# nkkrnkl/category-agnostic-pose-estimation

Hardware: AMD Instinct MI355X
Metric: episodes/sec (1-shot, 256x256, 17kpt) training step (higher is better)
Workload: dtype f32 storage/accumulate, GEMMs as bf16x3 split (3 bf16 MFMAs per product); 1 GPU; configs[1]: 1-shot training step (fwd+loss+bwd+clip+AdamW at learning rate 0, dropout on), 256x256, 17 kpt, ResNet-50 + deformable transformer, 16 episodes x 2 queries per GPU; episodes_per_gpu=16, queries_per_episode=2, image_size=256, global_batch_episodes=16, parallelism=dp1, weights=random init (no checkpoint offline)

## Files before the change

category-agnostic-pose-estimation_amd/csrc/msda.hip:

```cpp
#include <stdlib.h>
#include "common.h"

namespace {

struct Levels {
  int H[4], W[4], start[4];
};

constexpr int HEADS = 8, HD = 32, CH = HEADS * HD;

__device__ __forceinline__ int sel4(const int (&a)[4], int l) { return l == 0 ? a[0] : (l == 1 ? a[1] : (l == 2 ? a[2] : a[3])); }

__global__ void __launch_bounds__(256) msda_fwd_kernel(const float* __restrict__ value, const float* __restrict__ offw,
                                                        const float* __restrict__ ref, float* __restrict__ out,
                                                        Levels lv, int N, int S, int Lq, int L, int P, int blocks_per_image) {
  const int lane = threadIdx.x & 63, wv = threadIdx.x >> 6;
  int n, chunk;
  {
    const int b = blockIdx.x;
    const int xcd = b & 7, loc = b >> 3;
    const int imgs_per_x = (N + 7) >> 3;
    const int ii = loc / blocks_per_image;
    chunk = loc - ii * blocks_per_image;
    n = ii * 8 + xcd;
// ... 363 lines not shown
      const float top = v00.C + fx * dt, bot = v10.C + fx * db;                    \
      p_aw += go.C * (top + fy * (bot - top));                                     \
      p_x += go.C * (dt + fy * (db - dt));                                         \
      p_y += go.C * (bot - top);                                                   \
    }
    CAPE_TAP_CH(x) CAPE_TAP_CH(y) CAPE_TAP_CH(z) CAPE_TAP_CH(w)
#undef CAPE_TAP_CH
    const float r_aw = sum8(p_aw), r_x = sum8(p_x), r_y = sum8(p_y);
    if (i == (j & 7)) { daw[j >> 3] = r_aw; dpx[j >> 3] = r_x; dpy[j >> 3] = r_y; }
  }
  const float dot = sum8(aw[0] * daw[0] + aw[1] * daw[1]);
  float* dow = d_offw + qrow * rowlen;
#pragma unroll
  for (int s = 0; s < 2; ++s) {
    const int j = i + 8 * s;
    const bool live = j < LP;
    const float gx = aw[s] * dpx[s], gy = aw[s] * dpy[s];
    if (live) {
      *reinterpret_cast<float2*>(dow + (h * LP + j) * 2) = make_float2(gx, gy);
      dow[HEADS * LP * 2 + h * LP + j] = aw[s] * (daw[s] - dot);
    }
    if (d_ref) {
      float rx = live ? gx * (float)sel4(lv.W, lev[s]) : 0.f;
      float ry = live ? gy * (float)sel4(lv.H, lev[s]) : 0.f;
      if (P == 4) {
        rx += dpp_f<0xB1>(rx); rx += dpp_f<0x4E>(rx);
        ry += dpp_f<0xB1>(ry); ry += dpp_f<0x4E>(ry);
        rx += __shfl_xor(rx, 8); rx += __shfl_xor(rx, 16); rx += __shfl_xor(rx, 32);
        ry += __shfl_xor(ry, 8); ry += __shfl_xor(ry, 16); ry += __shfl_xor(ry, 32);
        if (live && h == 0 && (i & 3) == 0) *reinterpret_cast<float2*>(&d_ref[(qrow * L + lev[s]) * 2]) = make_float2(rx, ry);
      } else if (live) {
        atomicAdd(&d_ref[(qrow * L + lev[s]) * 2 + 0], rx);
        atomicAdd(&d_ref[(qrow * L + lev[s]) * 2 + 1], ry);
      }
    }
  }
}

struct ValRec { uint2 ids; float4 w; };

template <int VC>
__global__ void __launch_bounds__(1024) msda_bwd_value_kernel(const float* __restrict__ d_out, const float* __restrict__ offw,
                                                              const float* __restrict__ ref, float* __restrict__ d_value,
                                                              Levels lv, int N, int S, int Lq, int L, int P) {
  constexpr int VS = VC, GROUPS = HD / VC, BPI = HEADS * GROUPS;
  constexpr int SLOTS = 64 / VC;
  extern __shared__ __attribute__((aligned(16))) double slab[];
  __shared__ uint2 rec_ids[16][64];
  __shared__ float4 rec_w[16][64];
  int n, sub;
  {
    const int b = blockIdx.x, xcd = b & 7, loc = b >> 3;
    n = (loc / BPI) * 8 + xcd;
    sub = loc % BPI;
    if (n >= N) return;
  }
  const int h = sub / GROUPS, grp = sub % GROUPS;
  for (int k = threadIdx.x; k < (S + 1) * VS; k += 1024) slab[k] = 0.0;
  __syncthreads();

  const int lane = threadIdx.x & 63, wv = threadIdx.x >> 6;
  const int g = lane >> 4, j = lane & 15;
  const int c = lane & (VC - 1), slot = lane / VC;
  static_assert(SLOTS * VC == 64 && 16 % VC == 0, "a slot's records must stay inside one query");
  const int LP = L * P;
  const int rowlen = HEADS * LP * 3;
// ... 182 lines not shown
    const int l = (int)(unsigned)wd;
    const int hh = (int)(unsigned)(wd >> 32) - (l >> 31);
    lo = finite ? (float)l * inv_scale : nanv;
    hi = finite ? (float)hh * inv_scale : nanv;
  };
  constexpr int Q = VP / 2;
  for (int k = threadIdx.x; k < S * Q; k += 1024) {
    const int p_ = k / Q, c2 = (k % Q) * 2;
    float4 o;
    dec(fslab[p_ * VP + c2], o.x, o.y);
    dec(fslab[p_ * VP + c2 + 1], o.z, o.w);
    *reinterpret_cast<float4*>(dvb + (long long)p_ * CH + c2 * 2) = o;
  }
}

int fill_levels(Levels& lv, const int* shapes, const int* level_start, int L, int S) {
  CAPE_REQUIRE(L >= 1 && L <= 4, "cape_msda: L=%d must be in 1..4", L);
  long long tot = 0;
  for (int l = 0; l < 4; ++l) {
    lv.H[l] = l < L ? shapes[2 * l] : 1;
    lv.W[l] = l < L ? shapes[2 * l + 1] : 1;
    lv.start[l] = l < L ? level_start[l] : 0;
    if (l < L) {
      CAPE_REQUIRE(lv.H[l] > 0 && lv.W[l] > 0 && lv.start[l] == tot, "cape_msda: level %d shape/start inconsistent", l);
      tot += (long long)lv.H[l] * lv.W[l];
    }
  }
  CAPE_REQUIRE(tot == S, "cape_msda: sum(H*W)=%lld != S=%d", tot, S);
  return 0;
}

}

extern "C" int cape_msda_fwd(const float* value, const float* offw, const float* ref, const int* shapes,
                             const int* level_start, float* out, int N, int S, int Lq, int L, int P,
                             cape_stream_t stream) {
  CAPE_REQUIRE(value && offw && ref && shapes && level_start && out, "cape_msda_fwd: null pointer");
  CAPE_REQUIRE(P >= 1 && L * P <= 16, "cape_msda_fwd: L*P=%d must be <= 16", L * P);
  if (N <= 0 || Lq <= 0) return 0;
  Levels lv;
  if (fill_levels(lv, shapes, level_start, L, S)) return 1;
  const int bpi = (Lq + 3) / 4;
  const int imgs_per_x = (N + 7) / 8;
  const long long blocks = (long long)imgs_per_x * bpi * 8;
  CAPE_REQUIRE(blocks < (1ll << 31), "cape_msda_fwd: grid too large");
  static const bool shuffle_form = getenv("CAPE_MSDA_FWD_SHUFFLE") != nullptr;
  if (S < 65535 && !shuffle_form)
    hipLaunchKernelGGL(msda_fwd_rec_kernel, dim3((unsigned)blocks), dim3(256), 0, as_stream(stream), value, offw, ref, out, lv,
                       N, S, Lq, L, P, bpi);
  else
    hipLaunchKernelGGL(msda_fwd_kernel, dim3((unsigned)blocks), dim3(256), 0, as_stream(stream), value, offw, ref, out, lv,
                       N, S, Lq, L, P, bpi);
  CAPE_LAUNCH_CHECK("cape_msda_fwd");
  return 0;
}

static int msda_bwd_check(const float* d_out, const float* value, const float* offw, const float* ref, const int* shapes,
                          const int* level_start, float* d_value, float* d_offw, int L, int P) {
  CAPE_REQUIRE(d_out && value && offw && ref && shapes && level_start && d_value && d_offw, "cape_msda_bwd: null pointer");
  CAPE_REQUIRE(P >= 1 && L * P <= 16, "cape_msda_bwd: L*P=%d must be <= 16", L * P);
  return 0;
}

extern "C" int cape_msda_bwd_atomic(const float* d_out, const float* value, const float* offw, const float* ref,
                                    const int* shapes, const int* level_start, float* d_value, float* d_offw, float* d_ref,
                                    int N, int S, int Lq, int L, int P, cape_stream_t stream) {
  if (msda_bwd_check(d_out, value, offw, ref, shapes, level_start, d_value, d_offw, L, P)) return 1;
  if (N <= 0 || Lq <= 0) return 0;
  Levels lv;
  if (fill_levels(lv, shapes, level_start, L, S)) return 1;
  hipError_t e = hipMemsetAsync(d_value, 0, sizeof(float) * (size_t)N * S * CH, as_stream(stream));
  if (e == hipSuccess && d_ref) e = hipMemsetAsync(d_ref, 0, sizeof(float) * (size_t)N * Lq * L * 2, as_stream(stream));
  if (e != hipSuccess) return cape_set_error("cape_msda_bwd_atomic: memset: %s", hipGetErrorString(e));
  const long long waves = (long long)N * Lq * 4;
  const long long blocks = (waves + 3) / 4;
  CAPE_REQUIRE(blocks < (1ll << 31), "cape_msda_bwd_atomic: grid too large");
  hipLaunchKernelGGL(msda_bwd_kernel, dim3((unsigned)blocks), dim3(256), 0, as_stream(stream), d_out, value, offw, ref,
                     d_value, d_offw, d_ref, lv, N, S, Lq, L, P, waves);
  CAPE_LAUNCH_CHECK("cape_msda_bwd_atomic");
  return 0;
}

extern "C" int cape_msda_bwd(const float* d_out, const float* value, const float* offw, const float* ref,
                             const int* shapes, const int* level_start, float* d_value, float* d_offw, float* d_ref,
                             int N, int S, int Lq, int L, int P, cape_stream_t stream) {
  return cape_msda_bwd_ex(d_out, value, offw, ref, shapes, level_start, d_value, d_offw, d_ref, N, S, Lq, L, P, 0, stream);
}

extern "C" int cape_msda_bwd_ex(const float* d_out, const float* value, const float* offw, const float* ref,
                                const int* shapes, const int* level_start, float* d_value, float* d_offw, float* d_ref,
                                int N, int S, int Lq, int L, int P, int value_accum, cape_stream_t stream) {
  CAPE_REQUIRE(value_accum == 0 || value_accum == 1, "cape_msda_bwd_ex: value_accum must be 0 (fp64 slab) or 1 (fixed-point pairs)");
  if (msda_bwd_check(d_out, value, offw, ref, shapes, level_start, d_value, d_offw, L, P)) return 1;
  if (N <= 0 || Lq <= 0) return 0;
  const size_t kMaxSlab = 160 * 1024 - 16 * 64 * (sizeof(uint4) + sizeof(float4)) - 512;
  int vc = 8;
  while (vc >= 2 && (size_t)(S + 1) * vc * sizeof(double) > kMaxSlab) vc >>= 1;
  const size_t slab_bytes = (size_t)(S + 1) * vc * sizeof(double);
  static const bool force_atomic = getenv("CAPE_MSDA_BWD_ATOMIC") != nullptr;
  const long long imgs8 = ((long long)N + 7) / 8;
  const int bpi = (Lq + 3) / 4;
  const long long vblocks = imgs8 * 8 * HEADS * (HD / (vc < 2 ? 2 : vc));
  if (force_atomic || vc < 2 || S >= 65535 || vblocks >= (1ll << 31) || imgs8 * 8 * bpi >= (1ll << 31))
    return cape_msda_bwd_atomic(d_out, value, offw, ref, shapes, level_start, d_value, d_offw, d_ref, N, S, Lq, L, P, stream);
  Levels lv;
  if (fill_levels(lv, shapes, level_start, L, S)) return 1;
  static bool attr_done = false;
  if (!attr_done) {
    hipError_t e = hipFuncSetAttribute(reinterpret_cast<const void*>(msda_bwd_value_kernel<8>),
                                       hipFuncAttributeMaxDynamicSharedMemorySize, (int)kMaxSlab);
    if (e == hipSuccess) e = hipFuncSetAttribute(reinterpret_cast<const void*>(msda_bwd_value_kernel<4>),
                                                 hipFuncAttributeMaxDynamicSharedMemorySize, (int)kMaxSlab);
    if (e == hipSuccess) e = hipFuncSetAttribute(reinterpret_cast<const void*>(msda_bwd_value_kernel<2>),
                                                 hipFuncAttributeMaxDynamicSharedMemorySize, (int)kMaxSlab);
    if (e == hipSuccess) e = hipFuncSetAttribute(reinterpret_cast<const void*>(msda_bwd_value_fx_kernel<8>),
                                                 hipFuncAttributeMaxDynamicSharedMemorySize, (int)kMaxSlab);
    if (e == hipSuccess) e = hipFuncSetAttribute(reinterpret_cast<const void*>(msda_bwd_value_fx_kernel<4>),
                                                 hipFuncAttributeMaxDynamicSharedMemorySize, (int)kMaxSlab);
    if (e == hipSuccess) e = hipFuncSetAttribute(reinterpret_cast<const void*>(msda_bwd_value_fx_kernel<2>),
                                                 hipFuncAttributeMaxDynamicSharedMemorySize, (int)kMaxSlab);
    if (e != hipSuccess) return cape_set_error("cape_msda_bwd: hipFuncSetAttribute: %s", hipGetErrorString(e));
    attr_done = true;
  }
  if (d_ref && P != 4) {
    hipError_t e = hipMemsetAsync(d_ref, 0, sizeof(float) * (size_t)N * Lq * L * 2, as_stream(stream));
    if (e != hipSuccess) return cape_set_error("cape_msda_bwd: memset: %s", hipGetErrorString(e));
  }
#define VALUE_LAUNCH(W)                                                                                                     \
  hipLaunchKernelGGL((msda_bwd_value_kernel<W>), dim3((unsigned)vblocks), dim3(1024), slab_bytes, as_stream(stream), d_out, offw, \
                     ref, d_value, lv, N, S, Lq, L, P)
#define VALUE_LAUNCH_FX(W)                                                                                                  \
  hipLaunchKernelGGL((msda_bwd_value_fx_kernel<W>), dim3((unsigned)fxblocks), dim3(1024), fx_bytes, as_stream(stream),           \
                     d_out, offw, ref, d_value, lv, N, S, Lq, L, P)
  if (value_accum == 1) {
    int vp = vc;
    while (vp > 2 && imgs8 * 8 * HEADS * (HD / (2 * vp)) < 256) vp >>= 1;
    const long long fxblocks = imgs8 * 8 * HEADS * (HD / (2 * vp));
    const size_t fx_bytes = (size_t)(S + 1) * vp * sizeof(unsigned long long);
    if (vp == 8) VALUE_LAUNCH_FX(8); else if (vp == 4) VALUE_LAUNCH_FX(4); else VALUE_LAUNCH_FX(2);
  } else {
    if (vc == 8) VALUE_LAUNCH(8); else if (vc == 4) VALUE_LAUNCH(4); else VALUE_LAUNCH(2);
  }
#undef VALUE_LAUNCH_FX
#undef VALUE_LAUNCH
  hipLaunchKernelGGL(msda_bwd_offw_kernel, dim3((unsigned)(imgs8 * 8 * bpi)), dim3(256), 0, as_stream(stream), d_out, value, offw,
                     ref, d_offw, d_ref, lv, N, S, Lq, L, P, bpi);
  CAPE_LAUNCH_CHECK("cape_msda_bwd");
  return 0;
}
```

category-agnostic-pose-estimation_amd/hip/lib.py:

```python
import ctypes
import os

import torch

from ctypes import POINTER, c_char_p, c_float, c_int, c_int32, c_int64, c_longlong, c_size_t, c_uint32, c_uint64, c_uint8, c_void_p

_HERE = os.path.dirname(os.path.abspath(__file__))
LIB_PATH = os.environ.get("CAPE_HIP_LIB", os.path.join(_HERE, "..", "csrc", "libcape_hip.so"))
LIB_PATH = os.path.abspath(LIB_PATH)

if not os.path.exists(LIB_PATH):
    raise ImportError(
        f"libcape_hip.so not found at {LIB_PATH}; build it with `python -c 'import __graft_entry__ as g; g.build()'` "
        "(or `make -C category-agnostic-pose-estimation_amd/csrc`).  There is no CPU fallback.")
try:
    _lib = ctypes.CDLL(LIB_PATH)
except OSError as e:
    raise ImportError(f"cannot load {LIB_PATH}: {e}") from e

_lib.cape_last_error.restype = c_char_p
_lib.cape_abi_version.restype = c_int


class GemmDesc(ctypes.Structure):
# ... 67 lines not shown
        "w_off", "b_off", "value", "w_mo", "b_mo", "ln1_g", "ln1_b",
        "w1", "b1", "w2", "b2", "ln3_g", "ln3_b", "m1w", "m1b", "m2w", "m2b", "m3w", "m3b")]


class DecodeStepDesc(ctypes.Structure):
    _fields_ = [
        ("N", c_int), ("n_layers", c_int), ("step", c_int), ("T", c_int), ("P", c_int), ("S", c_int), ("L", c_int),
        ("n_points", c_int), ("ncls", c_int), ("ffn_dim", c_int),
        ("shapes", c_int * 8), ("level_start", c_int * 4),
        ("emb", c_void_p), ("qpos0", c_void_p), ("refin0", c_void_p), ("ref0", c_void_p), ("vr", c_void_p), ("dim_t", c_void_p),
        ("class_w", c_void_p), ("class_b", c_void_p),
        ("pos_w", c_void_p), ("pos_b", c_void_p), ("pos_gamma", c_void_p), ("pos_beta", c_void_p),
        ("out_logits", c_void_p), ("ld_logits", c_longlong),
        ("out_coords", c_void_p), ("ld_coords", c_longlong),
        ("out_hs", c_void_p), ("ld_hs", c_longlong),
        ("layers", DecodeLayerDesc * DECODE_MAX_LAYERS),
    ]


P, I, LL, F, U32 = c_void_p, c_int, c_longlong, c_float, c_uint32
_SIGS = {
    "cape_rng_advance": [P, P],
    "cape_stream_fork": [P, P],
    "cape_stream_join": [P, P],
    "cape_gemm_f32": [POINTER(GemmDesc), P],
    "cape_gemm_group_f32": [POINTER(GemmDesc), I, I, P],
    "cape_pack_weights": [P, I, I, P],
    "cape_colsum_f32": [P, LL, I, LL, I, I, P, I, P],
    "cape_add_layernorm_fwd": [P, P, P, P, P, P, P, P, P, I, I, F, P, U32, P],
    "cape_add_layernorm_bwd": [P, P, P, P, P, P, P, P, P, P, P, I, I, F, P, U32, P],
    "cape_groupnorm_fwd": [P, P, P, P, LL, P, P, I, I, I, I, P, c_size_t, P],
    "cape_groupnorm_bwd": [P, LL, P, P, P, P, P, P, P, I, I, I, I, P, c_size_t, P],
    "cape_msda_fwd": [P, P, P, P, P, P, I, I, I, I, I, P],
    "cape_msda_bwd": [P, P, P, P, P, P, P, P, P, I, I, I, I, I, P],
    "cape_msda_bwd_ex": [P, P, P, P, P, P, P, P, P, I, I, I, I, I, I, P],
    "cape_msda_bwd_atomic": [P, P, P, P, P, P, P, P, P, I, I, I, I, I, P],
    "cape_attn_fwd": [P, P, P, P, P, LL, LL, LL, LL, LL, LL, LL, LL, I, I, I, I, F, I, I, P, F, P, U32, P],
    "cape_attn_bwd": [P, P, P, P, P, P, P, P, P, LL, LL, LL, LL, LL, LL, LL, LL, I, I, I, I, F, I, I, P, F, P, U32, P],
    "cape_flash_attn_fwd": [P, P, P, P, P, LL, LL, LL, LL, LL, LL, LL, LL, I, I, I, I, F, I, I, P, F, P, U32, P],
    "cape_flash_attn_bwd": [P, P, P, P, P, P, P, P, P, P, LL, LL, LL, LL, LL, LL, LL, LL, I, I, I, I, F, I, I, P, F, P, U32, P],
    "cape_attn_softmax_fwd": [P, P, P, I, I, I, I, F, I, I, P, F, P, U32, P],
    "cape_attn_softmax_bwd": [P, P, I, I, I, I, F, F, P, U32, P],
    "cape_add_f32": [P, P, P, LL, P],
    "cape_level_embed_add": [P, P, P, P, I, I, I, I, P],
    "cape_add_n_f32": [POINTER(c_void_p), I, P, LL, P],
    "cape_add_n_rows_f32": [POINTER(c_void_p), POINTER(c_longlong), I, P, LL, LL, I, P],
    "cape_augment_batch": [P, I, I, I, P, P, P],
    "cape_gelu_f32": [P, P, LL, P],
    "cape_support_masks": [P, P, P, I, I, I, P],
    "cape_interleave2x2_f32": [POINTER(c_void_p), P, P, I, I, I, I, P],
    "cape_gelu_bwd_f32": [P, P, P, LL, P],
    "cape_scale_residual_bwd_f32": [P, P, P, P, P, LL, I, P],
    "cape_scale_residual_f32": [P, P, P, P, LL, I, P],
    "cape_nchw_to_nhwc": [P, P, I, I, I, I, I, P],
    "cape_bn_fold": [P, P, P, P, F, P, P, I, P],
    "cape_maxpool3x3s2_nhwc": [P, P, I, I, I, I, P],
    "cape_bn_relu_bwd": [P, P, P, P, P, LL, I, I, P],
    "cape_affine_act_f32": [P, P, P, P, LL, I, I, P],
    "cape_relu_drop_bwd": [P, P, P, LL, F, P],
    "cape_pos_sine_level": [P, P, P, P, LL, I, I, I, I, P],
    "cape_token_embed_fwd": [P, P, P, P, P, P, P, P, P, P, LL, I, I, P],
    "cape_token_embed_bwd": [P, P, P, P, P, P, P, P, P, P, LL, I, I, I, P],
    "cape_query_sine_fwd": [P, P, P, LL, P],
    "cape_query_sine_bwd": [P, P, P, P, I, LL, P],
    "cape_refine_fwd": [P, P, P, LL, P],
    "cape_refine_bwd": [P, P, P, P, P, I, LL, P],
    "cape_sigmoid_fwd": [P, P, LL, P],
    "cape_sigmoid_bwd": [P, P, P, I, LL, P],
# ... 55 lines not shown
```

category-agnostic-pose-estimation_amd/hip/ops.py:

```python
import ctypes
import math
import os
import weakref

import torch

from . import lib

_F32 = torch.float32


_raw_stream = getattr(torch._C, "_cuda_getCurrentRawStream", None)
_raw_device = getattr(torch._C, "_cuda_getDevice", None)


_side = [None]


def raw_current_stream():
    if _raw_stream is not None and _raw_device is not None:
        return _raw_stream(_raw_device())
    return torch.cuda.current_stream().cuda_stream


# ... 400 lines not shown
    assert x.numel() == N * HW * C
    mean = torch.empty(N * G, dtype=_F32, device=x.device)
    rstd = torch.empty(N * G, dtype=_F32, device=x.device)
    ws, nbytes = _gn_workspace(N, C, G, x.device)
    lib.call("cape_groupnorm_fwd", _p(x), _p(gamma), _p(beta), _p(out), out_image_stride, _p(mean), _p(rstd), N, HW, C, G,
             _p(ws), nbytes, _stream())
    return mean, rstd


def groupnorm_bwd(d_out, d_out_image_stride, x, gamma, mean, rstd, dgamma, dbeta, N, HW, C, G=32):
    _chk(d_out, "gn_bwd.d_out", contiguous=False)
    d_x = torch.empty_like(x)
    ws, nbytes = _gn_workspace(N, C, G, x.device)
    lib.call("cape_groupnorm_bwd", _p(d_out), d_out_image_stride, _p(x), _p(gamma), _p(mean), _p(rstd), _p(d_x),
             _p(dgamma), _p(dbeta), N, HW, C, G, _p(ws), nbytes, _stream())
    return d_x


class LevelGeometry:

    def __init__(self, shapes):
        self.shapes = [(int(h), int(w)) for h, w in shapes]
        self.L = len(self.shapes)
        starts, s = [], 0
        for h, w in self.shapes:
            starts.append(s)
            s += h * w
        self.S = s
        self.starts = starts
        self._shapes_c = (ctypes.c_int * (2 * self.L))(*[v for hw in self.shapes for v in hw])
        self._starts_c = (ctypes.c_int * self.L)(*starts)


def msda_fwd(value, offw, ref, geo, N, Lq, P=4):
    for t, n in ((value, "value"), (offw, "offw"), (ref, "ref")):
        _chk(t, "msda." + n)
    assert value.numel() == N * geo.S * 256 and offw.numel() == N * Lq * 8 * geo.L * P * 3
    assert ref.numel() == N * Lq * geo.L * 2
    out = torch.empty(N, Lq, 256, dtype=_F32, device=value.device)
    lib.call("cape_msda_fwd", _p(value), _p(offw), _p(ref), geo._shapes_c, geo._starts_c, _p(out), N, geo.S, Lq, geo.L, P,
             _stream())
    return out


MSDA_VALUE_ACCUM = os.environ.get("CAPE_MSDA_VALUE_ACCUM", "auto")


def msda_bwd(d_out, value, offw, ref, geo, N, Lq, P=4, need_ref_grad=True, form="split"):
    _chk(d_out, "msda_bwd.d_out")
    d_value = torch.empty_like(value)
    d_offw = torch.empty_like(offw)
    d_ref = torch.empty_like(ref) if need_ref_grad else None
    if form == "split":
        form = MSDA_VALUE_ACCUM if MSDA_VALUE_ACCUM != "auto" else ("f64" if GEMM_PRECISION == 0 else "fx")
    if form == "atomic":
        lib.call("cape_msda_bwd_atomic", _p(d_out), _p(value), _p(offw), _p(ref), geo._shapes_c, geo._starts_c, _p(d_value),
                 _p(d_offw), _p(d_ref), N, geo.S, Lq, geo.L, P, _stream())
    else:
        lib.call("cape_msda_bwd_ex", _p(d_out), _p(value), _p(offw), _p(ref), geo._shapes_c, geo._starts_c, _p(d_value),
                 _p(d_offw), _p(d_ref), N, geo.S, Lq, geo.L, P, {"f64": 0, "fx": 1}[form], _stream())
    return d_value, d_offw, d_ref


def _ld(t):
    assert t.stride(-1) == 1
    return t.stride(-2)


def _attn_views(tag, Q, K, V, N, H, Lq, Lk, flash):
    for t, n, L_ in ((Q, "Q", Lq), (K, "K", Lk), (V, "V", Lk)):
        _chk(t, tag + "." + n, contiguous=False)
        assert t.dim() == 3 and t.shape[0] == N and t.shape[1] >= L_ and t.shape[2] == H * 32
        if flash:
            assert t.stride(2) == 1 and t.stride(1) % 4 == 0 and t.stride(0) % 4 == 0 and t.data_ptr() % 16 == 0
        assert _avail(t) >= (N - 1) * t.stride(0) + (L_ - 1) * t.stride(1) + H * 32


def _rng_ptr(rng, dropout_p):
    return rng.ptr if (rng is not None and dropout_p > 0) else None


def _attn_tail(Q, K, V, N, H, Lq, Lk, scale, mask_mode, causal_offset, kpm, dropout_p, rng, rng_stream):
    return (_ld(Q), _ld(K), _ld(V), H * 32, Q.stride(0), K.stride(0), V.stride(0), Lq * H * 32, N, H, Lq, Lk, float(scale), mask_mode,
            causal_offset, _p(kpm), float(dropout_p), _rng_ptr(rng, dropout_p), rng_stream, _stream())


def _attn_fwd(flash, Q, K, V, N, H, Lq, Lk, scale, mask_mode, causal_offset, kpm, dropout_p, rng, rng_stream):
    tag = "flash_attn" if flash else "attn"
    _attn_views(tag, Q, K, V, N, H, Lq, Lk, flash)
    if kpm is not None:
        _chk(kpm, tag + ".kpm", dtype=torch.uint8)
        assert kpm.numel() == N * Lk
    O = torch.empty(N, Lq, H * 32, dtype=_F32, device=Q.device)
# ... 765 lines not shown
```

include/cape_hip.h:

```cpp
#ifndef CAPE_HIP_H
#define CAPE_HIP_H

#include <stddef.h>
#include <stdint.h>

#ifdef __cplusplus
extern "C" {
#endif

typedef void* cape_stream_t;

const char* cape_last_error(void);
int cape_abi_version(void);

int cape_rng_advance(uint64_t* rng_state, cape_stream_t stream);

int cape_stream_fork(cape_stream_t main_stream, cape_stream_t side_stream);
int cape_stream_join(cape_stream_t main_stream, cape_stream_t side_stream);

typedef struct {
  int M, N, K;
  int a_mode, b_mode;
  const float* A; long long lda;
  const float* B; long long ldb;
// ... 85 lines not shown
  const float* vr;
  const float* dim_t;
  const float *class_w, *class_b;
  const float *pos_w, *pos_b, *pos_gamma, *pos_beta;
  float* out_logits; long long ld_logits;
  float* out_coords; long long ld_coords;
  float* out_hs; long long ld_hs;
  cape_decode_layer_desc layers[CAPE_DECODE_MAX_LAYERS];
} cape_decode_step_desc;
int cape_decode_step(const cape_decode_step_desc* d, cape_stream_t stream);

int cape_add_layernorm_fwd(const float* x, const float* y, const float* gamma, const float* beta,
                           float* out, float* mean, float* rstd, const float* pos, float* out_pos,
                           int rows, int C, float dropout_p, const uint64_t* rng_state, uint32_t rng_stream,
                           cape_stream_t stream);
int cape_add_layernorm_bwd(const float* d_out, const float* d_out_pos, const float* x, const float* y,
                           const float* gamma, const float* mean, const float* rstd,
                           float* d_x, float* d_y, float* dgamma, float* dbeta,
                           int rows, int C, float dropout_p, const uint64_t* rng_state, uint32_t rng_stream,
                           cape_stream_t stream);

size_t cape_groupnorm_workspace_bytes(int N, int C, int G);
int cape_groupnorm_fwd(const float* x, const float* gamma, const float* beta, float* out,
                       long long out_image_stride, float* mean, float* rstd,
                       int N, int HW, int C, int G, void* workspace, size_t workspace_bytes, cape_stream_t stream);
int cape_groupnorm_bwd(const float* d_out, long long d_out_image_stride, const float* x,
                       const float* gamma, const float* mean, const float* rstd,
                       float* d_x, float* dgamma, float* dbeta, int N, int HW, int C, int G,
                       void* workspace, size_t workspace_bytes, cape_stream_t stream);

int cape_msda_fwd(const float* value, const float* offw, const float* ref, const int* shapes,
                  const int* level_start, float* out, int N, int S, int Lq, int L, int P,
                  cape_stream_t stream);
int cape_msda_bwd(const float* d_out, const float* value, const float* offw, const float* ref,
                  const int* shapes, const int* level_start, float* d_value, float* d_offw, float* d_ref,
                  int N, int S, int Lq, int L, int P, cape_stream_t stream);
int cape_msda_bwd_ex(const float* d_out, const float* value, const float* offw, const float* ref,
                     const int* shapes, const int* level_start, float* d_value, float* d_offw, float* d_ref,
                     int N, int S, int Lq, int L, int P, int value_accum, cape_stream_t stream);
int cape_msda_bwd_atomic(const float* d_out, const float* value, const float* offw, const float* ref,
                         const int* shapes, const int* level_start, float* d_value, float* d_offw, float* d_ref,
                         int N, int S, int Lq, int L, int P, cape_stream_t stream);

int cape_attn_fwd(const float* Q, const float* K, const float* V, float* O, float* lse,
                  long long ldq, long long ldk, long long ldv, long long ldo,
                  long long bsq, long long bsk, long long bsv, long long bso,
                  int N, int H, int Lq, int Lk, float scale, int mask_mode, int causal_offset,
                  const uint8_t* kpm, float dropout_p, const uint64_t* rng_state, uint32_t rng_stream,
                  cape_stream_t stream);
int cape_attn_bwd(const float* dO, const float* Q, const float* K, const float* V, const float* O,
                  const float* lse, float* dQ, float* dK, float* dV,
                  long long ldq, long long ldk, long long ldv, long long ldo,
                  long long bsq, long long bsk, long long bsv, long long bso,
                  int N, int H, int Lq, int Lk, float scale, int mask_mode, int causal_offset,
                  const uint8_t* kpm, float dropout_p, const uint64_t* rng_state, uint32_t rng_stream,
                  cape_stream_t stream);
int cape_attn_softmax_fwd(const float* S, float* P, float* Pd, int N, int H, int Lq, int Lk, float scale, int mask_mode,
                          int causal_offset, const uint8_t* kpm, float dropout_p, const uint64_t* rng_state,
                          uint32_t rng_stream, cape_stream_t stream);
int cape_attn_softmax_bwd(const float* P, float* dS, int N, int H, int Lq, int Lk, float scale, float dropout_p,
                          const uint64_t* rng_state, uint32_t rng_stream, cape_stream_t stream);

int cape_flash_attn_fwd(const float* Q, const float* K, const float* V, float* O, float* lse, long long ldq, long long ldk,
                        long long ldv, long long ldo, long long bsq, long long bsk, long long bsv, long long bso, int N, int H,
                        int Lq, int Lk, float scale, int mask_mode, int causal_offset, const uint8_t* kpm, float dropout_p,
                        const uint64_t* rng_state, uint32_t rng_stream, cape_stream_t stream);
int cape_flash_attn_bwd(const float* dO, const float* Q, const float* K, const float* V, const float* O, const float* lse,
                        float* dQ, float* dK, float* dV, float* d_ws, long long ldq, long long ldk, long long ldv, long long ldo,
                        long long bsq, long long bsk, long long bsv, long long bso, int N, int H, int Lq, int Lk, float scale,
                        int mask_mode, int causal_offset, const uint8_t* kpm, float dropout_p, const uint64_t* rng_state,
                        uint32_t rng_stream, cape_stream_t stream);

// ... 129 lines not shown
```

Baseline: 654.4 episodes/s.

## Add LDS-slab gather kernels for MSDA forward and offset-weight backward

Adds forward and offset/attention-weight backward kernels that stage the coarse levels of the value tensor for one (image, head) into shared memory. Taps on those levels are then read from LDS, while the finer levels are still gathered from global memory. A planner picks the split level under an LDS budget and sizes query chunks to fill the grid. The forward routes automatically when Lq is large enough and no reference gradient is needed. The backward slab path stays opt-in through an environment variable, and the change costs LDS occupancy plus extra launch-planning code.

```diff
diff --git a/category-agnostic-pose-estimation_amd/csrc/msda.hip b/category-agnostic-pose-estimation_amd/csrc/msda.hip
--- a/category-agnostic-pose-estimation_amd/csrc/msda.hip
+++ b/category-agnostic-pose-estimation_amd/csrc/msda.hip
@@ -419,6 +419,269 @@
       } else if (live) {
         atomicAdd(&d_ref[(qrow * L + lev[s]) * 2 + 0], rx);
         atomicAdd(&d_ref[(qrow * L + lev[s]) * 2 + 1], ry);
+      }
+    }
+  }
+}
+
+constexpr int SLAB_THREADS = 512, SLAB_WAVES = SLAB_THREADS / 64, SLAB_QPT = 8;
+constexpr int SLAB_STRIDE = 36;
+constexpr int GB = 4, GBB = 1;
+constexpr size_t SLAB_BUDGET = 52 * 1024;
+
+struct SlabGeo { int l0, row0, rows, ng, chunks, qchunk; };
+
+__device__ __forceinline__ bool slab_block(int N, const SlabGeo& sg, int& n, int& h, int& chunk) {
+  const int b = blockIdx.x, xcd = b & 7, loc = b >> 3;
+  const int per_img = HEADS * sg.chunks;
+  const int ii = loc / per_img, rem = loc - ii * per_img;
+  h = rem / sg.chunks;
+  chunk = rem - h * sg.chunks;
+  n = ii * 8 + xcd;
+  return n < N;
+}
+
+__device__ __forceinline__ void slab_fill(float* slab, const float* __restrict__ value, int n, int h, int S, const SlabGeo& sg) {
+  const float* src = value + ((long long)n * S + sg.row0) * CH + h * HD;
+  for (int k = threadIdx.x; k < sg.rows * 8; k += SLAB_THREADS) {
+    const int r = k >> 3, c = k & 7;
+    *reinterpret_cast<float4*>(slab + r * SLAB_STRIDE + c * 4) = *reinterpret_cast<const float4*>(src + (long long)r * CH + c * 4);
+  }
+  if (threadIdx.x < 8) *reinterpret_cast<float4*>(slab + sg.rows * SLAB_STRIDE + threadIdx.x * 4) = make_float4(0.f, 0.f, 0.f, 0.f);
+  __syncthreads();
+}
+
+__device__ __forceinline__ unsigned slab_id(unsigned id, bool in_slab, int S, const SlabGeo& sg) {
+  return in_slab ? (id >= (unsigned)S ? (unsigned)sg.rows : id - (unsigned)sg.row0) : id;
+}
+
+__global__ void __launch_bounds__(SLAB_THREADS) __attribute__((amdgpu_waves_per_eu(4, 4))) msda_fwd_slab_kernel(const float* __restrict__ value, const float* __restrict__ offw,
+                                                                     const float* __restrict__ ref, float* __restrict__ out,
+                                                                     Levels lv, SlabGeo sg, int N, int S, int Lq, int L, int P) {
+  extern __shared__ __attribute__((aligned(16))) float vslab[];
+  __shared__ uint2 rec_ids[SLAB_WAVES][SLAB_QPT * 16];
+  __shared__ float4 rec_w[SLAB_WAVES][SLAB_QPT * 16];
+  int n, h, chunk;
+  if (!slab_block(N, sg, n, h, chunk)) return;
+  slab_fill(vslab, value, n, h, S, sg);
+  const int lane = threadIdx.x & 63, wv = threadIdx.x >> 6;
+  const int qs = lane >> 3, i = lane & 7;
+  const int LP = L * P;
+  const int qend = min(Lq, (chunk + 1) * sg.qchunk);
+  int W[2], H[2], st[2], lev[2];
+#pragma unroll
+  for (int s = 0; s < 2; ++s) {
+    const int j = i + 8 * s;
+    lev[s] = j < LP ? j / P : 0;
+    W[s] = j < LP ? sel4(lv.W, lev[s]) : 1; H[s] = j < LP ? sel4(lv.H, lev[s]) : 1; st[s] = j < LP ? sel4(lv.start, lev[s]) : 0;
+  }
+  const float* vb = value + (long long)n * S * CH + h * HD + i * 4;
+  const float* sb = vslab + i * 4;
+  const uint2* rid = &rec_ids[wv][qs * 16];
+  const float4* rw = &rec_w[wv][qs * 16];
+  for (int qb = chunk * sg.qchunk + wv * SLAB_QPT; qb < qend; qb += SLAB_WAVES * SLAB_QPT) {
+    const int q = qb + qs;
+    const long long qrow = (long long)n * Lq + min(q, Lq - 1);
+    const float* ow = offw + qrow * (HEADS * LP * 3);
+    float px[2], py[2], lg[2];
+#pragma unroll
+    for (int s = 0; s < 2; ++s) {
+      const int j = i + 8 * s;
+      px[s] = 0.f; py[s] = 0.f; lg[s] = -INFINITY;
+      if (j < LP) {
+        const float2 rr = *reinterpret_cast<const float2*>(ref + (qrow * L + lev[s]) * 2);
+        const float2 oo = *reinterpret_cast<const float2*>(ow + (h * LP + j) * 2);
+        const float Wf = (float)W[s], Hf = (float)H[s];
+        px[s] = (rr.x + oo.x / Wf) * Wf - 0.5f;
+        py[s] = (rr.y + oo.y / Hf) * Hf - 0.5f;
+        lg[s] = ow[HEADS * LP * 2 + h * LP + j];
+      }
+    }
+    const float mx = max8(fmaxf(lg[0], lg[1]));
+    const float e0 = __expf(lg[0] - mx), e1 = __expf(lg[1] - mx);
+    const float inv = 1.f / sum8(e0 + e1);
+    const float aw[2] = {e0 * inv, e1 * inv};
+#pragma unroll
+    for (int s = 0; s < 2; ++s) {
+      const int j = i + 8 * s;
+      const Tap t = make_tap(px[s], py[s], W[s], H[s], st[s], j < LP, S);
+      const bool in_slab = j >= sg.ng;
+      const unsigned cl = (unsigned)(S - 1);
+      float4 w = make_float4(aw[s] * (1.f - t.fx) * (1.f - t.fy), aw[s] * t.fx * (1.f - t.fy), aw[s] * (1.f - t.fx) * t.fy,
+                             aw[s] * t.fx * t.fy);
+      if (t.i00 >= (unsigned)S) w.x = 0.f;
+      if (t.i01 >= (unsigned)S) w.y = 0.f;
+      if (t.i10 >= (unsigned)S) w.z = 0.f;
+      if (t.i11 >= (unsigned)S) w.w = 0.f;
+      const unsigned a = in_slab ? slab_id(t.i00, true, S, sg) : min(t.i00, cl), b = in_slab ? slab_id(t.i01, true, S, sg) : min(t.i01, cl);
+      const unsigned c = in_slab ? slab_id(t.i10, true, S, sg) : min(t.i10, cl), d = in_slab ? slab_id(t.i11, true, S, sg) : min(t.i11, cl);
+      rec_ids[wv][qs * 16 + j] = make_uint2(a | (b << 16), c | (d << 16));
+      rec_w[wv][qs * 16 + j] = w;
+    }
+    float4 acc = make_float4(0.f, 0.f, 0.f, 0.f);
+    auto consume = [&](const float4& w, const float4& c0, const float4& c1, const float4& c2, const float4& c3) {
+      acc.x += w.x * c0.x + w.y * c1.x + w.z * c2.x + w.w * c3.x;
+      acc.y += w.x * c0.y + w.y * c1.y + w.z * c2.y + w.w * c3.y;
+      acc.z += w.x * c0.z + w.y * c1.z + w.z * c2.z + w.w * c3.z;
+      acc.w += w.x * c0.w + w.y * c1.w + w.z * c2.w + w.w * c3.w;
+    };
+    auto sload = [&](int j, float4& w, float4 (&c)[4]) {
+      const uint2 ids = rid[j];
+      c[0] = *reinterpret_cast<const float4*>(sb + (ids.x & 0xFFFFu) * (unsigned)SLAB_STRIDE);
+      c[1] = *reinterpret_cast<const float4*>(sb + (ids.x >> 16) * (unsigned)SLAB_STRIDE);
+      c[2] = *reinterpret_cast<const float4*>(sb + (ids.y & 0xFFFFu) * (unsigned)SLAB_STRIDE);
+      c[3] = *reinterpret_cast<const float4*>(sb + (ids.y >> 16) * (unsigned)SLAB_STRIDE);
+      w = rw[j];
+    };
+    float4 cw, cc[4];
+    for (int j0 = 0; j0 < sg.ng; j0 += GB) {
+      float4 v[GB][4];
+#pragma unroll
+      for (int k = 0; k < GB; ++k) {
+        const uint2 ids = rid[min(j0 + k, sg.ng - 1)];
+        v[k][0] = *reinterpret_cast<const float4*>(vb + (ids.x & 0xFFFFu) * (unsigned)CH);
+        v[k][1] = *reinterpret_cast<const float4*>(vb + (ids.x >> 16) * (unsigned)CH);
+        v[k][2] = *reinterpret_cast<const float4*>(vb + (ids.y & 0xFFFFu) * (unsigned)CH);
+        v[k][3] = *reinterpret_cast<const float4*>(vb + (ids.y >> 16) * (unsigned)CH);
+      }
+#pragma unroll
+      for (int k = 0; k < GB; ++k)
+        if (j0 + k < sg.ng) consume(rw[j0 + k], v[k][0], v[k][1], v[k][2], v[k][3]);
+    }
+    sload(sg.ng, cw, cc);
+    for (int j = sg.ng; j < LP; ++j) {
+      float4 nw, nc[4];
+      sload(min(j + 1, LP - 1), nw, nc);
+      consume(cw, cc[0], cc[1], cc[2], cc[3]);
+      cw = nw; cc[0] = nc[0]; cc[1] = nc[1]; cc[2] = nc[2]; cc[3] = nc[3];
+    }
+    if (q < Lq) *reinterpret_cast<float4*>(out + qrow * CH + h * HD + i * 4) = acc;
+  }
+}
+
+__global__ void __launch_bounds__(SLAB_THREADS) __attribute__((amdgpu_waves_per_eu(4, 4))) msda_bwd_offw_slab_kernel(const float* __restrict__ d_out, const float* __restrict__ value,
+                                                                          const float* __restrict__ offw, const float* __restrict__ ref,
+                                                                          float* __restrict__ d_offw, Levels lv, SlabGeo sg, int N, int S,
+                                                                          int Lq, int L, int P) {
+  extern __shared__ __attribute__((aligned(16))) float vslab[];
+  __shared__ uint4 recs[SLAB_WAVES][SLAB_QPT * 16];
+  int n, h, chunk;
+  if (!slab_block(N, sg, n, h, chunk)) return;
+  slab_fill(vslab, value, n, h, S, sg);
+  const int lane = threadIdx.x & 63, wv = threadIdx.x >> 6;
+  const int qs = lane >> 3, i = lane & 7;
+  const int LP = L * P;
+  const int rowlen = HEADS * LP * 3;
+  const int qend = min(Lq, (chunk + 1) * sg.qchunk);
+  int W[2], H[2], st[2];
+#pragma unroll
+  for (int s = 0; s < 2; ++s) {
+    const int j = i + 8 * s;
+    const int l = j < LP ? j / P : 0;
+    W[s] = j < LP ? sel4(lv.W, l) : 1; H[s] = j < LP ? sel4(lv.H, l) : 1; st[s] = j < LP ? sel4(lv.start, l) : 0;
+  }
+  const float* vb = value + (long long)n * S * CH + h * HD + i * 4;
+  const float* sb = vslab + i * 4;
+  const uint4* myrec = &recs[wv][qs * 16];
+  for (int qb = chunk * sg.qchunk + wv * SLAB_QPT; qb < qend; qb += SLAB_WAVES * SLAB_QPT) {
+    const int q = qb + qs;
+    const long long qrow = (long long)n * Lq + min(q, Lq - 1);
+    const float* ow = offw + qrow * rowlen;
+    float lg[2], aw[2];
+#pragma unroll
+    for (int s = 0; s < 2; ++s) {
+      const int j = i + 8 * s;
+      const bool live = j < LP;
+      float px = 0.f, py = 0.f;
+      lg[s] = -INFINITY;
+      if (live) {
+        const int l = j / P;
+        const float2 rr = *reinterpret_cast<const float2*>(ref + (qrow * L + l) * 2);
+        const float2 oo = *reinterpret_cast<const float2*>(ow + (h * LP + j) * 2);
+        const float Wf = (float)W[s], Hf = (float)H[s];
+        px = (rr.x + oo.x / Wf) * Wf - 0.5f;
+        py = (rr.y + oo.y / Hf) * Hf - 0.5f;
+        lg[s] = ow[HEADS * LP * 2 + h * LP + j];
+      }
+      const Tap t = make_tap(px, py, W[s], H[s], st[s], live, S);
+      const bool in_slab = j >= sg.ng;
+      recs[wv][qs * 16 + j] = make_uint4(slab_id(t.i00, in_slab, S, sg) | (slab_id(t.i01, in_slab, S, sg) << 16),
+                                         slab_id(t.i10, in_slab, S, sg) | (slab_id(t.i11, in_slab, S, sg) << 16),
+                                         __float_as_uint(t.fx), __float_as_uint(t.fy));
+    }
+    {
+      const float mx = max8(fmaxf(lg[0], lg[1]));
+      const float e0 = __expf(lg[0] - mx), e1 = __expf(lg[1] - mx);
+      const float inv = 1.f / sum8(e0 + e1);
+      aw[0] = e0 * inv; aw[1] = e1 * inv;
+    }
+    const float4 go = *reinterpret_cast<const float4*>(d_out + qrow * CH + h * HD + i * 4);
+    float daw[2] = {0.f, 0.f}, dpx[2] = {0.f, 0.f}, dpy[2] = {0.f, 0.f};
+    auto consume = [&](int j, float fx, float fy, const float4& v00, const float4& v01, const float4& v10, const float4& v11) {
+      float p_aw = 0.f, p_x = 0.f, p_y = 0.f;
+#define CAPE_TAP_CH(C)                                                             \
+      {                                                                            \
+        const float dt = v01.C - v00.C, db = v11.C - v10.C;                        \
+        const float top = v00.C + fx * dt, bot = v10.C + fx * db;                  \
+        p_aw += go.C * (top + fy * (bot - top));                                   \
+        p_x += go.C * (dt + fy * (db - dt));                                       \
+        p_y += go.C * (bot - top);                                                 \
+      }
+      CAPE_TAP_CH(x) CAPE_TAP_CH(y) CAPE_TAP_CH(z) CAPE_TAP_CH(w)
+#undef CAPE_TAP_CH
+      const float r_aw = sum8(p_aw), r_x = sum8(p_x), r_y = sum8(p_y);
+      const bool mine = i == (j & 7), hi = j >= 8;
+      if (mine && !hi) { daw[0] = r_aw; dpx[0] = r_x; dpy[0] = r_y; }
+      if (mine && hi) { daw[1] = r_aw; dpx[1] = r_x; dpy[1] = r_y; }
+    };
+    auto sload = [&](int j, uint4& r, float4 (&c)[4]) {
+      r = myrec[j];
+      c[0] = *reinterpret_cast<const float4*>(sb + (r.x & 0xFFFFu) * (unsigned)SLAB_STRIDE);
+      c[1] = *reinterpret_cast<const float4*>(sb + (r.x >> 16) * (unsigned)SLAB_STRIDE);
+      c[2] = *reinterpret_cast<const float4*>(sb + (r.y & 0xFFFFu) * (unsigned)SLAB_STRIDE);
+      c[3] = *reinterpret_cast<const float4*>(sb + (r.y >> 16) * (unsigned)SLAB_STRIDE);
+    };
+    const int ns = LP - sg.ng, nb = (sg.ng + GBB - 1) / GBB;
+    int js = sg.ng;
+    uint4 cr;
+    float4 cc[4];
+    sload(js, cr, cc);
+    for (int b = 0; b < nb; ++b) {
+      const int j0 = b * GBB;
+      uint4 ra[GBB];
+      float4 v[GBB][4];
+#pragma unroll
+      for (int k = 0; k < GBB; ++k) {
+        ra[k] = myrec[min(j0 + k, sg.ng - 1)];
+        const unsigned ids[4] = {ra[k].x & 0xFFFFu, ra[k].x >> 16, ra[k].y & 0xFFFFu, ra[k].y >> 16};
+#pragma unroll
+        for (int c = 0; c < 4; ++c) {
+          const unsigned idc = min(ids[c], (unsigned)(S - 1));
+          const float4 x = *reinterpret_cast<const float4*>(vb + idc * (unsigned)CH);
+          v[k][c] = ids[c] < (unsigned)S ? x : make_float4(0.f, 0.f, 0.f, 0.f);
+        }
+      }
+      const int jend = sg.ng + (ns * (b + 1)) / nb;
+      for (; js < jend; ++js) {
+        uint4 nr;
+        float4 nc[4];
+        sload(min(js + 1, LP - 1), nr, nc);
+        consume(js, __uint_as_float(cr.z), __uint_as_float(cr.w), cc[0], cc[1], cc[2], cc[3]);
+        cr = nr; cc[0] = nc[0]; cc[1] = nc[1]; cc[2] = nc[2]; cc[3] = nc[3];
+      }
+#pragma unroll
+      for (int k = 0; k < GBB; ++k)
+        if (j0 + k < sg.ng)
+          consume(j0 + k, __uint_as_float(ra[k].z), __uint_as_float(ra[k].w), v[k][0], v[k][1], v[k][2], v[k][3]);
+    }
+    const float dot = sum8(aw[0] * daw[0] + aw[1] * daw[1]);
+    float* dow = d_offw + qrow * rowlen;
+#pragma unroll
+    for (int s = 0; s < 2; ++s) {
+      const int j = i + 8 * s;
+      if (j < LP && q < Lq) {
+        *reinterpret_cast<float2*>(dow + (h * LP + j) * 2) = make_float2(aw[s] * dpx[s], aw[s] * dpy[s]);
+        dow[HEADS * LP * 2 + h * LP + j] = aw[s] * (daw[s] - dot);
       }
     }
   }
@@ -667,16 +930,102 @@
 
 }
 
+constexpr int SLAB_MIN_LQ = 64;
+constexpr int SLAB_GRID_SLOTS = 512;
+
+static int slab_plan(const Levels& lv, int L, int P, int S, int N, int Lq, SlabGeo& sg) {
+  if (L < 2 || P < 1 || L * P > 16 || S >= 65535 || N <= 0 || Lq <= 0) return 0;
+  for (int l0 = 1; l0 < L; ++l0) {
+    const int rows = S - lv.start[l0];
+    if ((size_t)(rows + 1) * SLAB_STRIDE * sizeof(float) > SLAB_BUDGET) continue;
+    const long long pairs = (((long long)N + 7) / 8) * 8 * HEADS;
+    long long chunks = (SLAB_GRID_SLOTS + pairs - 1) / pairs;
+    const long long max_chunks = ((long long)Lq + SLAB_WAVES * SLAB_QPT - 1) / (SLAB_WAVES * SLAB_QPT);
+    if (chunks > max_chunks) chunks = max_chunks;
+    if (chunks < 1) chunks = 1;
+    const int qchunk = (int)(((Lq + chunks - 1) / chunks + SLAB_QPT - 1) / SLAB_QPT) * SLAB_QPT;
+    sg.l0 = l0; sg.row0 = lv.start[l0]; sg.rows = rows; sg.ng = l0 * P;
+    sg.qchunk = qchunk; sg.chunks = (Lq + qchunk - 1) / qchunk;
+    if (pairs * sg.chunks >= (1ll << 31)) return 0;
+    return l0;
+  }
+  return 0;
+}
+
+static int slab_attr() {
+  static bool done = false;
+  if (done) return 0;
+  hipError_t e = hipFuncSetAttribute(reinterpret_cast<const void*>(msda_fwd_slab_kernel), hipFuncAttributeMaxDynamicSharedMemorySize,
+                                     (int)SLAB_BUDGET);
+  if (e == hipSuccess) e = hipFuncSetAttribute(reinterpret_cast<const void*>(msda_bwd_offw_slab_kernel),
+                                               hipFuncAttributeMaxDynamicSharedMemorySize, (int)SLAB_BUDGET);
+  if (e != hipSuccess) return cape_set_error("cape_msda: hipFuncSetAttribute: %s", hipGetErrorString(e));
+  done = true;
+  return 0;
+}
+
+static int gather_route(const char* who, const Levels& lv, int L, int P, int S, int N, int Lq, bool has_d_ref, int gather_form,
+                        SlabGeo& sg) {
+  if (gather_form < 0 || gather_form > 2) { cape_set_error("%s: gather_form must be 0 (auto), 1 (record) or 2 (slab)", who); return -1; }
+  if (gather_form == 1) return 1;
+  const int l0 = has_d_ref ? 0 : slab_plan(lv, L, P, S, N, Lq, sg);
+  if (gather_form == 2) {
+    if (l0 == 0) {
+      cape_set_error("%s: the slab gather form cannot run here (needs L >= 2, L*P <= 16, S < 65535, a level >= 1 whose rest fits "
+                     "the LDS budget, and no d_ref); L=%d P=%d S=%d d_ref=%d", who, L, P, S, (int)has_d_ref);
+      return -1;
+    }
+    return 2;
+  }
+  return (l0 != 0 && Lq >= SLAB_MIN_LQ) ? 2 : 1;
+}
+
+extern "C" int cape_msda_gather_plan(const int* shapes, int L, int P, int N, int Lq, int has_d_ref, int* l0_out) {
+  if (l0_out) *l0_out = 0;
+  if (!shapes || L < 1 || L > 4) return 1;
+  Levels lv;
+  int start[4] = {0, 0, 0, 0};
+  long long tot = 0;
+  for (int l = 0; l < L; ++l) {
+    if (shapes[2 * l] <= 0 || shapes[2 * l + 1] <= 0) return 1;
+    start[l] = (int)tot;
+    tot += (long long)shapes[2 * l] * shapes[2 * l + 1];
+    if (tot >= 65535) return 1;
+  }
+  if (fill_levels(lv, shapes, start, L, (int)tot)) return 1;
+  SlabGeo sg = {};
+  const int form = gather_route("cape_msda_gather_plan", lv, L, P, (int)tot, N, Lq, has_d_ref != 0, 0, sg);
+  if (form == 2 && l0_out) *l0_out = sg.l0;
+  return form == 2 ? 2 : 1;
+}
+
 extern "C" int cape_msda_fwd(const float* value, const float* offw, const float* ref, const int* shapes,
                              const int* level_start, float* out, int N, int S, int Lq, int L, int P,
                              cape_stream_t stream) {
+  return cape_msda_fwd_ex(value, offw, ref, shapes, level_start, out, N, S, Lq, L, P, 0, stream);
+}
+
+extern "C" int cape_msda_fwd_ex(const float* value, const float* offw, const float* ref, const int* shapes,
+                                const int* level_start, float* out, int N, int S, int Lq, int L, int P, int gather_form,
+                                cape_stream_t stream) {
   CAPE_REQUIRE(value && offw && ref && shapes && level_start && out, "cape_msda_fwd: null pointer");
   CAPE_REQUIRE(P >= 1 && L * P <= 16, "cape_msda_fwd: L*P=%d must be <= 16", L * P);
   if (N <= 0 || Lq <= 0) return 0;
   Levels lv;
   if (fill_levels(lv, shapes, level_start, L, S)) return 1;
+  SlabGeo sg = {};
+  const int form = gather_route("cape_msda_fwd", lv, L, P, S, N, Lq, false, gather_form, sg);
+  if (form < 0) return 1;
   const int bpi = (Lq + 3) / 4;
   const int imgs_per_x = (N + 7) / 8;
+  if (form == 2) {
+    if (slab_attr()) return 1;
+    const size_t bytes = (size_t)(sg.rows + 1) * SLAB_STRIDE * sizeof(float);
+    hipLaunchKernelGGL(msda_fwd_slab_kernel, dim3((unsigned)(imgs_per_x * 8 * HEADS * sg.chunks)), dim3(SLAB_THREADS), bytes,
+                       as_stream(stream), value, offw, ref, out, lv, sg, N, S, Lq, L, P);
+    CAPE_LAUNCH_CHECK("cape_msda_fwd");
+    return 0;
+  }
   const long long blocks = (long long)imgs_per_x * bpi * 8;
   CAPE_REQUIRE(blocks < (1ll << 31), "cape_msda_fwd: grid too large");
   static const bool shuffle_form = getenv("CAPE_MSDA_FWD_SHUFFLE") != nullptr;
@@ -719,13 +1068,21 @@
 extern "C" int cape_msda_bwd(const float* d_out, const float* value, const float* offw, const float* ref,
                              const int* shapes, const int* level_start, float* d_value, float* d_offw, float* d_ref,
                              int N, int S, int Lq, int L, int P, cape_stream_t stream) {
-  return cape_msda_bwd_ex(d_out, value, offw, ref, shapes, level_start, d_value, d_offw, d_ref, N, S, Lq, L, P, 0, stream);
+  return cape_msda_bwd_form(d_out, value, offw, ref, shapes, level_start, d_value, d_offw, d_ref, N, S, Lq, L, P, 0, 0, stream);
 }
 
 extern "C" int cape_msda_bwd_ex(const float* d_out, const float* value, const float* offw, const float* ref,
                                 const int* shapes, const int* level_start, float* d_value, float* d_offw, float* d_ref,
                                 int N, int S, int Lq, int L, int P, int value_accum, cape_stream_t stream) {
+  return cape_msda_bwd_form(d_out, value, offw, ref, shapes, level_start, d_value, d_offw, d_ref, N, S, Lq, L, P, value_accum, 0,
+                            stream);
+}
+
+extern "C" int cape_msda_bwd_form(const float* d_out, const float* value, const float* offw, const float* ref,
+                                  const int* shapes, const int* level_start, float* d_value, float* d_offw, float* d_ref,
+                                  int N, int S, int Lq, int L, int P, int value_accum, int gather_form, cape_stream_t stream) {
   CAPE_REQUIRE(value_accum == 0 || value_accum == 1, "cape_msda_bwd_ex: value_accum must be 0 (fp64 slab) or 1 (fixed-point pairs)");
+  CAPE_REQUIRE(gather_form >= 0 && gather_form <= 2, "cape_msda_bwd: gather_form must be 0 (auto), 1 (record) or 2 (slab)");
   if (msda_bwd_check(d_out, value, offw, ref, shapes, level_start, d_value, d_offw, L, P)) return 1;
   if (N <= 0 || Lq <= 0) return 0;
   const size_t kMaxSlab = 160 * 1024 - 16 * 64 * (sizeof(uint4) + sizeof(float4)) - 512;
@@ -736,10 +1093,18 @@
   const long long imgs8 = ((long long)N + 7) / 8;
   const int bpi = (Lq + 3) / 4;
   const long long vblocks = imgs8 * 8 * HEADS * (HD / (vc < 2 ? 2 : vc));
-  if (force_atomic || vc < 2 || S >= 65535 || vblocks >= (1ll << 31) || imgs8 * 8 * bpi >= (1ll << 31))
+  if (force_atomic || vc < 2 || S >= 65535 || vblocks >= (1ll << 31) || imgs8 * 8 * bpi >= (1ll << 31)) {
+    CAPE_REQUIRE(gather_form != 2, "cape_msda_bwd: the slab gather form cannot run where the backward takes memory-side atomics");
     return cape_msda_bwd_atomic(d_out, value, offw, ref, shapes, level_start, d_value, d_offw, d_ref, N, S, Lq, L, P, stream);
+  }
   Levels lv;
   if (fill_levels(lv, shapes, level_start, L, S)) return 1;
+  SlabGeo sg = {};
+  static const char* bwd_gather_env = getenv("CAPE_MSDA_BWD_GATHER");
+  int gform = gather_route("cape_msda_bwd", lv, L, P, S, N, Lq, d_ref != nullptr, gather_form, sg);
+  if (gform < 0) return 1;
+  if (gather_form == 0 && gform == 2 && !(bwd_gather_env && bwd_gather_env[0] == 's')) gform = 1;
+  if (gform == 2 && slab_attr()) return 1;
   static bool attr_done = false;
   if (!attr_done) {
     hipError_t e = hipFuncSetAttribute(reinterpret_cast<const void*>(msda_bwd_value_kernel<8>),
@@ -778,8 +1143,13 @@
   }
 #undef VALUE_LAUNCH_FX
 #undef VALUE_LAUNCH
-  hipLaunchKernelGGL(msda_bwd_offw_kernel, dim3((unsigned)(imgs8 * 8 * bpi)), dim3(256), 0, as_stream(stream), d_out, value, offw,
-                     ref, d_offw, d_ref, lv, N, S, Lq, L, P, bpi);
+  if (gform == 2)
+    hipLaunchKernelGGL(msda_bwd_offw_slab_kernel, dim3((unsigned)(imgs8 * 8 * HEADS * sg.chunks)), dim3(SLAB_THREADS),
+                       (size_t)(sg.rows + 1) * SLAB_STRIDE * sizeof(float), as_stream(stream), d_out, value, offw, ref, d_offw, lv, sg,
+                       N, S, Lq, L, P);
+  else
+    hipLaunchKernelGGL(msda_bwd_offw_kernel, dim3((unsigned)(imgs8 * 8 * bpi)), dim3(256), 0, as_stream(stream), d_out, value, offw,
+                       ref, d_offw, d_ref, lv, N, S, Lq, L, P, bpi);
   CAPE_LAUNCH_CHECK("cape_msda_bwd");
   return 0;
 }
diff --git a/category-agnostic-pose-estimation_amd/hip/lib.py b/category-agnostic-pose-estimation_amd/hip/lib.py
--- a/category-agnostic-pose-estimation_amd/hip/lib.py
+++ b/category-agnostic-pose-estimation_amd/hip/lib.py
@@ -123,8 +123,11 @@
     "cape_groupnorm_fwd": [P, P, P, P, LL, P, P, I, I, I, I, P, c_size_t, P],
     "cape_groupnorm_bwd": [P, LL, P, P, P, P, P, P, P, I, I, I, I, P, c_size_t, P],
     "cape_msda_fwd": [P, P, P, P, P, P, I, I, I, I, I, P],
+    "cape_msda_fwd_ex": [P, P, P, P, P, P, I, I, I, I, I, I, P],
     "cape_msda_bwd": [P, P, P, P, P, P, P, P, P, I, I, I, I, I, P],
     "cape_msda_bwd_ex": [P, P, P, P, P, P, P, P, P, I, I, I, I, I, I, P],
+    "cape_msda_bwd_form": [P, P, P, P, P, P, P, P, P, I, I, I, I, I, I, I, P],
+    "cape_msda_gather_plan": [P, I, I, I, I, I, P],
     "cape_msda_bwd_atomic": [P, P, P, P, P, P, P, P, P, I, I, I, I, I, P],
     "cape_attn_fwd": [P, P, P, P, P, LL, LL, LL, LL, LL, LL, LL, LL, I, I, I, I, F, I, I, P, F, P, U32, P],
     "cape_attn_bwd": [P, P, P, P, P, P, P, P, P, LL, LL, LL, LL, LL, LL, LL, LL, I, I, I, I, F, I, I, P, F, P, U32, P],
diff --git a/category-agnostic-pose-estimation_amd/hip/ops.py b/category-agnostic-pose-estimation_amd/hip/ops.py
--- a/category-agnostic-pose-estimation_amd/hip/ops.py
+++ b/category-agnostic-pose-estimation_amd/hip/ops.py
@@ -456,21 +456,24 @@
         self._starts_c = (ctypes.c_int * self.L)(*starts)
 
 
-def msda_fwd(value, offw, ref, geo, N, Lq, P=4):
+_MSDA_GATHER = {"auto": 0, "record": 1, "slab": 2}
+
+
+def msda_fwd(value, offw, ref, geo, N, Lq, P=4, gather="auto"):
     for t, n in ((value, "value"), (offw, "offw"), (ref, "ref")):
         _chk(t, "msda." + n)
     assert value.numel() == N * geo.S * 256 and offw.numel() == N * Lq * 8 * geo.L * P * 3
     assert ref.numel() == N * Lq * geo.L * 2
     out = torch.empty(N, Lq, 256, dtype=_F32, device=value.device)
-    lib.call("cape_msda_fwd", _p(value), _p(offw), _p(ref), geo._shapes_c, geo._starts_c, _p(out), N, geo.S, Lq, geo.L, P,
-             _stream())
+    lib.call("cape_msda_fwd_ex", _p(value), _p(offw), _p(ref), geo._shapes_c, geo._starts_c, _p(out), N, geo.S, Lq, geo.L, P,
+             _MSDA_GATHER[gather], _stream())
     return out
 
 
 MSDA_VALUE_ACCUM = os.environ.get("CAPE_MSDA_VALUE_ACCUM", "auto")
 
 
-def msda_bwd(d_out, value, offw, ref, geo, N, Lq, P=4, need_ref_grad=True, form="split"):
+def msda_bwd(d_out, value, offw, ref, geo, N, Lq, P=4, need_ref_grad=True, form="split", gather="auto"):
     _chk(d_out, "msda_bwd.d_out")
     d_value = torch.empty_like(value)
     d_offw = torch.empty_like(offw)
@@ -478,11 +481,12 @@
     if form == "split":
         form = MSDA_VALUE_ACCUM if MSDA_VALUE_ACCUM != "auto" else ("f64" if GEMM_PRECISION == 0 else "fx")
     if form == "atomic":
+        assert gather != "slab", "msda_bwd: the atomic form has no slab gather kernel"
         lib.call("cape_msda_bwd_atomic", _p(d_out), _p(value), _p(offw), _p(ref), geo._shapes_c, geo._starts_c, _p(d_value),
                  _p(d_offw), _p(d_ref), N, geo.S, Lq, geo.L, P, _stream())
     else:
-        lib.call("cape_msda_bwd_ex", _p(d_out), _p(value), _p(offw), _p(ref), geo._shapes_c, geo._starts_c, _p(d_value),
-                 _p(d_offw), _p(d_ref), N, geo.S, Lq, geo.L, P, {"f64": 0, "fx": 1}[form], _stream())
+        lib.call("cape_msda_bwd_form", _p(d_out), _p(value), _p(offw), _p(ref), geo._shapes_c, geo._starts_c, _p(d_value),
+                 _p(d_offw), _p(d_ref), N, geo.S, Lq, geo.L, P, {"f64": 0, "fx": 1}[form], _MSDA_GATHER[gather], _stream())
     return d_value, d_offw, d_ref
 
 
diff --git a/include/cape_hip.h b/include/cape_hip.h
--- a/include/cape_hip.h
+++ b/include/cape_hip.h
@@ -141,12 +141,19 @@
 int cape_msda_fwd(const float* value, const float* offw, const float* ref, const int* shapes,
                   const int* level_start, float* out, int N, int S, int Lq, int L, int P,
                   cape_stream_t stream);
+int cape_msda_fwd_ex(const float* value, const float* offw, const float* ref, const int* shapes,
+                     const int* level_start, float* out, int N, int S, int Lq, int L, int P, int gather_form,
+                     cape_stream_t stream);
+int cape_msda_gather_plan(const int* shapes, int L, int P, int N, int Lq, int has_d_ref, int* l0_out);
 int cape_msda_bwd(const float* d_out, const float* value, const float* offw, const float* ref,
                   const int* shapes, const int* level_start, float* d_value, float* d_offw, float* d_ref,
                   int N, int S, int Lq, int L, int P, cape_stream_t stream);
 int cape_msda_bwd_ex(const float* d_out, const float* value, const float* offw, const float* ref,
                      const int* shapes, const int* level_start, float* d_value, float* d_offw, float* d_ref,
                      int N, int S, int Lq, int L, int P, int value_accum, cape_stream_t stream);
+int cape_msda_bwd_form(const float* d_out, const float* value, const float* offw, const float* ref,
+                       const int* shapes, const int* level_start, float* d_value, float* d_offw, float* d_ref,
+                       int N, int S, int Lq, int L, int P, int value_accum, int gather_form, cape_stream_t stream);
 int cape_msda_bwd_atomic(const float* d_out, const float* value, const float* offw, const float* ref,
                          const int* shapes, const int* level_start, float* d_value, float* d_offw, float* d_ref,
                          int N, int S, int Lq, int L, int P, cape_stream_t stream);
```

Result: slower. 610.2 episodes/s (-6.8%).
